# Itseez/opencv

Measured on AMD Instinct MI355X. Metric: Mpix/s per GPU (4K CV_8U Gaussian5x5) + achieved HBM GB/s vs roofline, 1/2/4/8 GPUs, higher is better.
Workload: dtype u8; 1 GPU; cv::GaussianBlur 5x5 sigma=0 BORDER_REFLECT_101 on 3840x2160 CV_8UC1, 9216 device-resident frames per GPU per step (152.9 GB of HBM: one pass = 18 launches of 512 frames); frames_per_gpu=9216, frames_per_launch=512, ranks=1, collective=none (1 GPU)

## Files before the change

opencv_amd/csrc/smooth.hip:

```cpp
#include "rt.h"
#include "gausskernel.h"
#include "seproll.h"
#include "seplong.h"
#include "sepmx.h"
#include <cstring>
#include <cstdlib>

using namespace mi355;

namespace {

struct FixedTaps { uint16_t kx[33]; uint16_t ky[33]; int nx, ny; };

__global__ __launch_bounds__(256) void k_sepfixed_generic(
    const uchar* __restrict__ src, size_t sstep, size_t sframe,
    uchar* __restrict__ dst, size_t dstep, size_t dframe,
    int W, int H, int cn, int mL, int mT, int mR, int mB, int border, FixedTaps t)
{
    const int b = blockIdx.x * 64 + (threadIdx.x & 63);
    const int y = blockIdx.y * 4 + (threadIdx.x >> 6);
    if (b >= W * cn || y >= H) return;
    src += (size_t)blockIdx.z * sframe;
    dst += (size_t)blockIdx.z * dframe;
    const int x = b / cn, c = b - x * cn;
// ... 119 lines not shown
                Hrow[k] = a + (b << 2) + (m << 1) + (m << 2); }
            {   uint32_t a = pairAt<1, -2 * CN, HD>(E, O, k) + pairAt<1, 2 * CN, HD>(E, O, k);
                uint32_t b = pairAt<1, -CN, HD>(E, O, k) + pairAt<1, CN, HD>(E, O, k);
                uint32_t m = pairAt<1, 0, HD>(E, O, k);
                Hrow[4 + k] = a + (b << 2) + (m << 1) + (m << 2); }
        } else {
            Hrow[k]     = pairAt<0, -CN, HD>(E, O, k) + pairAt<0, CN, HD>(E, O, k) + (pairAt<0, 0, HD>(E, O, k) << 1);
            Hrow[4 + k] = pairAt<1, -CN, HD>(E, O, k) + pairAt<1, CN, HD>(E, O, k) + (pairAt<1, 0, HD>(E, O, k) << 1);
        }
    }
}

template <int KS, int CN>
__global__ __launch_bounds__(256) void k_binomial_roll(
    const uchar* __restrict__ src, size_t sstep, size_t sframe,
    uchar* __restrict__ dst, size_t dstep, size_t dframe,
    int W, int H, int nchunks, int segRows, int border)
{
    constexpr int R = KS / 2, HD = RollCfg<KS, CN>::HD;
    const int lane = threadIdx.x & 63;
    const int c = (blockIdx.x * 4 + (threadIdx.x >> 6)) * 64 + lane;
    const int y0 = blockIdx.y * segRows;
    const int y1 = min(H, y0 + segRows);
    src += (size_t)blockIdx.z * sframe;
    dst += (size_t)blockIdx.z * dframe;
    const bool active = c < nchunks;

    uint32_t Hw[KS][8];
    {
        RawRow<HD> pre[KS - 1];
#pragma unroll
        for (int i = 0; i < KS - 1; i++) loadRow<KS, CN>(pre[i], src, sstep, y0 - R + i, W, H, c, nchunks, lane, border);
#pragma unroll
        for (int i = 0; i < KS - 1; i++) hfilter<KS, CN>(Hw[i], pre[i], c, nchunks, lane);
    }
    for (int y = y0; y < y1; y += KS) {
        RawRow<HD> raw[KS];
#pragma unroll
        for (int u = 0; u < KS; u++)
            if (y + u < y1) loadRow<KS, CN>(raw[u], src, sstep, y + u + R, W, H, c, nchunks, lane, border);
#pragma unroll
        for (int u = 0; u < KS; u++) {
            if (y + u < y1) {
                hfilter<KS, CN>(Hw[(KS - 1 + u) % KS], raw[u], c, nchunks, lane);
                uint32_t o[4];
                if constexpr (KS == 5) {
                    const uint32_t* h0 = Hw[(u + 0) % 5]; const uint32_t* h1 = Hw[(u + 1) % 5];
                    const uint32_t* h2 = Hw[(u + 2) % 5]; const uint32_t* h3 = Hw[(u + 3) % 5];
                    const uint32_t* h4 = Hw[(u + 4) % 5];
                    uint32_t v[8];
#pragma unroll
                    for (int i = 0; i < 8; i++) {
                        const uint32_t b4 = lshlAdd(h1[i] + h3[i] + h2[i], 2, 0x00800080u);
                        v[i] = h0[i] + h4[i] + lshlAdd(h2[i], 1, b4);
                    }
#pragma unroll
                    for (int k = 0; k < 4; k++) o[k] = __builtin_amdgcn_perm(v[4 + k], v[k], 0x07030501u);
                } else {
                    const uint32_t* h0 = Hw[(u + 0) % 3]; const uint32_t* h1 = Hw[(u + 1) % 3]; const uint32_t* h2 = Hw[(u + 2) % 3];
#pragma unroll
                    for (int k = 0; k < 4; k++) {
                        uint32_t ve = ((h0[k] + h2[k] + (h1[k] << 1) + 0x00080008u) >> 4) & 0x00FF00FFu;
                        uint32_t vo = ((h0[4 + k] + h2[4 + k] + (h1[4 + k] << 1) + 0x00080008u) >> 4) & 0x00FF00FFu;
                        o[k] = ve | (vo << 8);
                    }
                }
                if (active)
                    *reinterpret_cast<uint4*>(dst + (size_t)(y + u) * dstep + 16 * (size_t)c) = make_uint4(o[0], o[1], o[2], o[3]);
            }
        }
    }
}

template <int HD> struct RawRow2 {
    uint4 m;
    uint32_t side[HD];
};

template <int HD> struct EdgeSel {
    uint32_t la[HD], lb[HD], lc[HD];
    uint32_t ra[HD], rb[HD], rc[HD];
};

__device__ __forceinline__ void selSetByte(uint32_t& a, uint32_t& b, uint32_t& c, int j, int idx )
{
    const uint32_t sh = 8u * (uint32_t)j, clr = ~(0xffu << sh);
    uint32_t va = 0x0cu, vb = 0x0cu, vc = 0x0cu;
    if (idx >= 8)      { vb = (uint32_t)(idx - 8); vc = 4u + (uint32_t)j; }
    else if (idx >= 0) { va = (uint32_t)idx;       vc = (uint32_t)j; }
    a = (a & clr) | (va << sh); b = (b & clr) | (vb << sh); c = (c & clr) | (vc << sh);
}

__device__ __forceinline__ uint32_t gather16(const uint4& m, uint32_t a, uint32_t b, uint32_t c)
{
    const uint32_t t1 = __builtin_amdgcn_perm(m.y, m.x, a);
    const uint32_t t2 = __builtin_amdgcn_perm(m.w, m.z, b);
    return __builtin_amdgcn_perm(t2, t1, c);
}

template <int KS, int CN, bool NTL = false>
__device__ __forceinline__ void issueRow(RawRow2<RollCfg<KS, CN>::HD>& r, const uchar* __restrict__ row, int mainOff, int sideOff)
{
    constexpr int HD = RollCfg<KS, CN>::HD;
    if constexpr (NTL) {
        typedef uint32_t u32x4 __attribute__((ext_vector_type(4)));
        u32x4 v = __builtin_nontemporal_load(reinterpret_cast<const u32x4*>(row + mainOff));
        r.m = make_uint4(v.x, v.y, v.z, v.w);
    } else
    r.m = *reinterpret_cast<const uint4*>(row + mainOff);
#pragma unroll
    for (int d = 0; d < HD; d++) r.side[d] = *reinterpret_cast<const uint32_t*>(row + sideOff + 4 * d);
}

template <int KS, int CN, bool EB = true>
__device__ __forceinline__ void hfilter2(uint32_t (&Hrow)[8], const RawRow2<RollCfg<KS, CN>::HD>& r,
                                         bool hasFirst, bool hasLast, bool isLastChunk, const EdgeSel<RollCfg<KS, CN>::HD>& es)
{
    constexpr int HD = RollCfg<KS, CN>::HD;
    constexpr int NW = 4 + 2 * HD;
    uint32_t X[NW];
    const uint32_t mv[4] = {r.m.x, r.m.y, r.m.z, r.m.w};
    uint32_t hl[HD], hr[HD];
#pragma unroll
    for (int d = 0; d < HD; d++) { hl[d] = r.side[d]; hr[d] = r.side[d]; }
    if (hasFirst) {
#pragma unroll
        for (int d = 0; d < HD; d++) { hl[d] = gather16(r.m, es.la[d], es.lb[d], es.lc[d]); if constexpr (EB) asm volatile("" : "+v"(hl[d])); }
    }
    uint32_t hb[HD];
#pragma unroll
    for (int d = 0; d < HD; d++) hb[d] = 0;
    if (hasLast) {
#pragma unroll
        for (int d = 0; d < HD; d++) { hb[d] = gather16(r.m, es.ra[d], es.rb[d], es.rc[d]); if constexpr (EB) asm volatile("" : "+v"(hb[d])); }
    }
#pragma unroll
    for (int d = 0; d < HD; d++) {
        X[d] = __builtin_amdgcn_update_dpp(hl[d], mv[4 - HD + d], 0x138, 0xf, 0xf, false);
        uint32_t rr = __builtin_amdgcn_update_dpp(hr[d], mv[d], 0x130, 0xf, 0xf, false);
        if (hasLast) { rr = isLastChunk ? hb[d] : rr; if constexpr (EB) asm volatile("" : "+v"(rr)); }
        X[HD + 4 + d] = rr;
    }
#pragma unroll
    for (int d = 0; d < 4; d++) X[HD + d] = mv[d];
    uint32_t E[NW], O[NW];
#pragma unroll
    for (int d = 0; d < NW; d++) {
        E[d] = __builtin_amdgcn_perm(0u, X[d], 0x0c020c00u);
        O[d] = __builtin_amdgcn_perm(0u, X[d], 0x0c030c01u);
    }
#pragma unroll
    for (int k = 0; k < 4; k++) {
        if constexpr (KS == 5) {
            {   uint32_t a = pairAt<0, -2 * CN, HD>(E, O, k) + pairAt<0, 2 * CN, HD>(E, O, k);
                uint32_t b = pairAt<0, -CN, HD>(E, O, k) + pairAt<0, CN, HD>(E, O, k);
                uint32_t m = pairAt<0, 0, HD>(E, O, k);
                Hrow[k] = a + (b << 2) + (m << 1) + (m << 2); }
            {   uint32_t a = pairAt<1, -2 * CN, HD>(E, O, k) + pairAt<1, 2 * CN, HD>(E, O, k);
                uint32_t b = pairAt<1, -CN, HD>(E, O, k) + pairAt<1, CN, HD>(E, O, k);
                uint32_t m = pairAt<1, 0, HD>(E, O, k);
                Hrow[4 + k] = a + (b << 2) + (m << 1) + (m << 2); }
        } else {
            Hrow[k]     = pairAt<0, -CN, HD>(E, O, k) + pairAt<0, CN, HD>(E, O, k) + (pairAt<0, 0, HD>(E, O, k) << 1);
            Hrow[4 + k] = pairAt<1, -CN, HD>(E, O, k) + pairAt<1, CN, HD>(E, O, k) + (pairAt<1, 0, HD>(E, O, k) << 1);
        }
    }
}
// ... 105 lines not shown
            for (int k = 0; k < 4; k++) o[k] = __builtin_amdgcn_perm(v[4 + k], v[k], 0x07030501u);
        } else {
            const uint32_t* h0 = Hw[(u + 0) % 3]; const uint32_t* h1 = Hw[(u + 1) % 3]; const uint32_t* h2 = Hw[(u + 2) % 3];
#pragma unroll
            for (int k = 0; k < 4; k++) {
                uint32_t ve = ((h0[k] + h2[k] + (h1[k] << 1) + 0x00080008u) >> 4) & 0x00FF00FFu;
                uint32_t vo = ((h0[4 + k] + h2[4 + k] + (h1[4 + k] << 1) + 0x00080008u) >> 4) & 0x00FF00FFu;
                o[k] = ve | (vo << 8);
            }
        }
        if (active) {
            typedef uint32_t u32x4 __attribute__((ext_vector_type(4)));
            u32x4 ov = {o[0], o[1], o[2], o[3]};
            u32x4* dp = reinterpret_cast<u32x4*>(dst + (size_t)gy(j) * dstep + 16 * (size_t)c);
            if constexpr (NT) __builtin_nontemporal_store(ov, dp);
            else *dp = ov;
        }
    };
    if constexpr (RING) {
        RawRow2<HD> pre[KS - 1];
        int pvalid[KS - 1];
#pragma unroll
        for (int i = 0; i < KS - 1; i++) {
            const int ry = rowIdx(gy(min(i - R, nrows - 1 + R)));
            pvalid[i] = ry >= 0;
            issueRow<KS, CN>(pre[i], src + (size_t)max(ry, 0) * sstep, mainOff, sideOff);
            __builtin_amdgcn_sched_barrier(0);
        }
#pragma unroll
        for (int u = 0; u < KS; u++) {
            refill(u, u + R);
            __builtin_amdgcn_sched_barrier(0);
        }
#pragma unroll
        for (int i = 0; i < KS - 1; i++) {
            hfilter2<KS, CN, EB>(Hw[i], pre[i], hasFirst, hasLast, isLastChunk, es);
#pragma unroll
            for (int j = 0; j < 8; j++) Hw[i][j] = pvalid[i] ? Hw[i][j] : 0u;
        }
        int y = 0;
        for (; y + KS <= nrows; y += KS) {
#pragma unroll
            for (int u = 0; u < KS; u++) {
                consume(u);
                refill(u, y + u + KS + R);
                emit(u, y + u);
            }
        }
#pragma unroll
        for (int u = 0; u < KS - 1; u++) {
            if (y + u < nrows) {
                consume(u);
                emit(u, y + u);
            }
        }
    } else {
#pragma unroll
        for (int i = 0; i < KS - 1; i++) {
            const int ry = rowIdx(gy(min(i - R, nrows - 1 + R)));
            if (ry < 0) {
#pragma unroll
                for (int j = 0; j < 8; j++) Hw[i][j] = 0;
            } else {
                RawRow2<HD> pre;
                issueRow<KS, CN>(pre, src + (size_t)ry * sstep, mainOff, sideOff);
                hfilter2<KS, CN, EB>(Hw[i], pre, hasFirst, hasLast, isLastChunk, es);
            }
        }
#pragma unroll
        for (int u = 0; u < KS; u++) refill(u, u + R);
        for (int y = 0; y < nrows; y += KS) {
#pragma unroll
            for (int u = 0; u < KS; u++) {
                if (y + u < nrows) {
                    consume(u);
                    refill(u, y + u + KS + R);
                    emit(u, y + u);
                }
            }
        }
    }
}

template <bool NT>
__global__ __launch_bounds__(256) void k_copy16(const uint4* __restrict__ s, uint4* __restrict__ d, size_t n16, int perThread)
{
    typedef uint32_t u32x4 __attribute__((ext_vector_type(4)));
    size_t base = ((size_t)blockIdx.x * perThread) * 256 + threadIdx.x;
#pragma unroll 4
    for (int i = 0; i < perThread; i++) {
        size_t j = base + (size_t)i * 256;
        if (j < n16) {
            uint4 v = s[j];
            u32x4 ov = {v.x, v.y, v.z, v.w};
            if constexpr (NT) __builtin_nontemporal_store(ov, reinterpret_cast<u32x4*>(d + j));
            else d[j] = v;
        }
    }
}

template <int UNROLL>
__global__ __launch_bounds__(256) void k_copy_colwalk(const uchar* __restrict__ src, uchar* __restrict__ dst, size_t step, size_t frame,
                                                      int H, int nchunks, int nstrips, int segRows, int nseg, int nframes)
{
    const int lane = threadIdx.x & 63;
    const int wid = __builtin_amdgcn_readfirstlane((int)(blockIdx.x * 4 + (threadIdx.x >> 6)));
    const int strip = wid % nstrips, t0 = wid / nstrips, seg = t0 % nseg, fr = t0 / nseg;
    if (fr >= nframes) return;
    const int c = strip * 64 + lane;
    if (c >= nchunks) return;
    const int y0 = seg * segRows, y1 = min(H, y0 + segRows);
    const uchar* s = src + (size_t)fr * frame + 16 * (size_t)c;
    uchar* d = dst + (size_t)fr * frame + 16 * (size_t)c;
    for (int y = y0; y < y1; y += UNROLL) {
        uint4 v[UNROLL];
#pragma unroll
        for (int u = 0; u < UNROLL; u++) v[u] = *reinterpret_cast<const uint4*>(s + (size_t)min(y + u, y1 - 1) * step);
#pragma unroll
        for (int u = 0; u < UNROLL; u++) if (y + u < y1) *reinterpret_cast<uint4*>(d + (size_t)(y + u) * step) = v[u];
    }
}


bool aligned16(const void* p, size_t step) { return (((uintptr_t)p | step) & 15) == 0; }

int envInt(const char* n, int d) { const char* v = getenv(n); return v ? atoi(v) : d; }

int& tuneSeg() { static int v = envInt("MI355CV_GAUSS_SEG", 0); return v; }
constexpr int kGaussVariantDefault = 6;
int& tuneVariant() { static int v = envInt("MI355CV_GAUSS_VARIANT", kGaussVariantDefault); return v; }

int& tuneAlt() { static int v = envInt("MI355CV_GAUSS_ALT", 1); return v; }
int& tuneLaunchWaves() { static int v = envInt("MI355CV_GAUSS_LAUNCH_WAVES", 393216); return v; }

template <int KS, int CN>
void launchRoll2(const uchar* s, size_t ss, size_t sf, uchar* d, size_t ds, size_t df, int nframes, int W, int H, int border, hipStream_t st, int nt)
{
    const int nchunks = W * CN / 16;
    const int nstrips = divUp(nchunks, 64);
    int seg = tuneSeg();
    if (seg <= 0) {
        long long per = (long long)nstrips * nframes;
        long long wantSeg = (2048 + per - 1) / per;
        seg = (int)((H + wantSeg - 1) / wantSeg);
        const int best = (nt == 4 && CN == 1) ? 12 : 16;
        if (seg > best) seg = best;
        if (seg < KS) seg = KS;
    }
    if (seg > H) seg = H;
    const int nseg = divUp(H, seg);
    const long long perFrame = (long long)nstrips * nseg;
    long long chunk = tuneLaunchWaves() > 0 ? (tuneLaunchWaves() + perFrame - 1) / perFrame : nframes;
    if (chunk < 1) chunk = 1;
    if (chunk > nframes) chunk = nframes;
    const int nlaunch = (int)((nframes + chunk - 1) / chunk);
    noteKernel("k_binomial_roll2<%d,%d,%s,false,%d,%s%s> grid=%u x256 seg=%d rows alt=%d, %d launch(es) of <= %lld frames", KS, CN, nt >= 1 ? "true" : "false", nt == 3 ? 6 : 4,
               nt == 2 ? "false" : "true", nt == 4 ? ",true" : "", (unsigned)((perFrame * chunk + 3) / 4), seg, tuneAlt(), nlaunch, chunk);
    for (long long f0 = 0; f0 < nframes; f0 += chunk) {
        const int nf = (int)(nframes - f0 < chunk ? nframes - f0 : chunk);
        const uchar* sp = s + (size_t)f0 * sf;
        uchar* dp = d + (size_t)f0 * df;
        dim3 grid((unsigned)((perFrame * nf + 3) / 4));
        if (nt >= 4)      hipLaunchKernelGGL((k_binomial_roll2<KS, CN, true, false, 4, true, true>), grid, dim3(256), 0, st, sp, ss, sf, dp, ds, df, W, H, nchunks, nstrips, seg, nseg, nf, border, tuneAlt());
        else if (nt == 3) hipLaunchKernelGGL((k_binomial_roll2<KS, CN, true, false, 6>), grid, dim3(256), 0, st, sp, ss, sf, dp, ds, df, W, H, nchunks, nstrips, seg, nseg, nf, border, tuneAlt());
        else if (nt == 2) hipLaunchKernelGGL((k_binomial_roll2<KS, CN, true, false, 4, false>), grid, dim3(256), 0, st, sp, ss, sf, dp, ds, df, W, H, nchunks, nstrips, seg, nseg, nf, border, tuneAlt());
        else if (nt == 1) hipLaunchKernelGGL((k_binomial_roll2<KS, CN, true, false, 4>), grid, dim3(256), 0, st, sp, ss, sf, dp, ds, df, W, H, nchunks, nstrips, seg, nseg, nf, border, tuneAlt());
        else              hipLaunchKernelGGL((k_binomial_roll2<KS, CN, false, false, 4>), grid, dim3(256), 0, st, sp, ss, sf, dp, ds, df, W, H, nchunks, nstrips, seg, nseg, nf, border, tuneAlt());
    }
}

template <int KS, int CN>
void launchRoll(const uchar* s, size_t ss, size_t sf, uchar* d, size_t ds, size_t df, int nframes, int W, int H, int border, hipStream_t st)
{
    const int nchunks = W * CN / 16;
    const int gx = divUp(nchunks, 256);
    const int segEnv = tuneSeg();
    int seg;
    if (segEnv > 0) seg = segEnv;
    else {
        long long stripsWaves = (long long)divUp(nchunks, 64) * nframes;
        long long wantSeg = (16384 + stripsWaves - 1) / stripsWaves;
        if (wantSeg < 1) wantSeg = 1;
        seg = (int)((H + wantSeg - 1) / wantSeg);
        if (seg < 4 * KS) seg = 4 * KS;
    }
    seg = divUp(seg, KS) * KS;
    if (seg > H) seg = divUp(H, KS) * KS;
    for (int f0 = 0; f0 < nframes; f0 += MAX_GRID_FRAMES) {
        dim3 grid(gx, divUp(H, seg), std::min(MAX_GRID_FRAMES, nframes - f0));
        hipLaunchKernelGGL((k_binomial_roll<KS, CN>), grid, dim3(256), 0, st, s + (size_t)f0 * sf, ss, sf, d + (size_t)f0 * df, ds, df, W, H, nchunks, seg, border);
    }
    noteKernel("k_binomial_roll<%d,%d> grid=%dx%dx%d x256 seg=%d rows, %d launch(es)", KS, CN, gx, divUp(H, seg), std::min(MAX_GRID_FRAMES, nframes), seg, divUp(nframes, MAX_GRID_FRAMES));
}

bool rollEligible(const uchar* s, size_t ss, size_t sf, const uchar* d, size_t ds, size_t df, int W, int H, int cn, int ks)
{
    if (ks != 3 && ks != 5) return false;
    if (cn < 1 || cn > 4) return false;
    if (!aligned16(s, ss) || !aligned16(d, ds) || (sf & 15) || (df & 15)) return false;
    if ((W * cn) % 16 != 0) return false;
    if (H < 1) return false;
    return true;
}

static int sepmxMinTaps()
{
    static const int v = std::getenv("MI355CV_SEPMX_MIN_TAPS") ? atoi(std::getenv("MI355CV_SEPMX_MIN_TAPS")) : 7;
    return v;
}

int runSmooth(const char* entry, const uchar* src, size_t sstep, size_t sframe, uchar* dst, size_t dstep, size_t dframe,
              int nframes, int W, int H, int cn, int mL, int mT, int mR, int mB,
              const uint16_t* kx, int nx, const uint16_t* ky, int ny, int border, bool binomial)
{
    MI355_DECLINE_IF(disabled());
    MI355_DECLINE_IF(W <= 0 || H <= 0 || nframes <= 0 || cn < 1 || cn > 4);
    MI355_DECLINE_IF(nx < 1 || ny < 1 || nx > lim::GAUSS8U_MAX_KSIZE || ny > lim::GAUSS8U_MAX_KSIZE || !(nx & 1) || !(ny & 1));
    MI355_DECLINE_IF(border < 0 || border > B_REFLECT_101);
    Stager stg;
    MI355_DECLINE_IF(!ensureDevice());
    const bool hostSrc = !isDevicePtr(src);
    MI355_DECLINE_IF(hostSrc && (size_t)W * H < minPixels());
    MI355_DECLINE_IF(!hostSrc && src == dst);

    size_t dss = 0, dds = 0;
    const size_t rowB = (size_t)W * cn;
    const uchar* dsrc; uchar* ddst;
    if (nframes == 1) {
        const uchar* top = src - (ptrdiff_t)mT * (ptrdiff_t)sstep - (ptrdiff_t)mL * cn;
        const uchar* dtop = stg.in(top, sstep, (size_t)(mL + W + mR) * cn, mT + H + mB, &dss);
        MI355_DECLINE_IF(!dtop);
        dsrc = dtop + (size_t)mT * dss + (size_t)mL * cn;
        ddst = stg.out(dst, dstep, rowB, H, &dds);
        MI355_DECLINE_IF(!ddst);
    } else {
        if (hostSrc || !isDevicePtr(dst)) return setError(MI355CV_NOT_IMPLEMENTED, "%s: batch entry needs device-resident frames", entry);
        dsrc = src; ddst = dst; dss = sstep; dds = dstep;
    }
    hipStream_t st = stream();
    const bool noMargins = !(mL | mT | mR | mB);
    if (binomial && noMargins && rollEligible(dsrc, dss, sframe, ddst, dds, dframe, W, H, cn, nx) && nx == ny) {
#define ROLL(KS_, CN_) do { if (tuneVariant() <= 1 || border == B_WRAP || W <= KS_ / 2) launchRoll<KS_, CN_>(dsrc, dss, sframe, ddst, dds, dframe, nframes, W, H, border, st); \
                            else launchRoll2<KS_, CN_>(dsrc, dss, sframe, ddst, dds, dframe, nframes, W, H, border, st, tuneVariant() - 2); } while (0)
        if (nx == 5) { switch (cn) { case 1: ROLL(5, 1); break; case 2: ROLL(5, 2); break; case 3: ROLL(5, 3); break; default: ROLL(5, 4); } }
        else         { switch (cn) { case 1: ROLL(3, 1); break; case 2: ROLL(3, 2); break; case 3: ROLL(3, 3); break; default: ROLL(3, 4); } }
#undef ROLL
    } else if (std::getenv("MI355CV_SMOOTH_GENERIC") == nullptr && std::max(nx, ny) >= sepmxMinTaps() && !(std::getenv("MI355CV_SEPMX") && std::getenv("MI355CV_SEPMX")[0] == '0') &&
               sepmxRun(stg, dsrc, dss, sframe, ddst, dds, dframe, nframes, W, H, cn, mL + W + mR, mT + H + mB, mL, mT, border, kx, nx, nx / 2, ky, ny, ny / 2, st)) {
    } else if (noMargins && std::getenv("MI355CV_SMOOTH_GENERIC") == nullptr &&
               seprollFixedSmooth(dsrc, dss, sframe, ddst, dds, dframe, nframes, W, H, cn, kx, nx, ky, ny, border, st)) {
    } else if (!noMargins && nframes == 1 && std::getenv("MI355CV_SMOOTH_GENERIC") == nullptr && [&] {
                   const Roi roi = {mL + W + mR, mT + H + mB, mL, mT};
                   return seprollFixedSmooth(dsrc, dss, 0, ddst, dds, 0, 1, W, H, cn, kx, nx, ky, ny, border, st, &roi); }()) {
    } else if (std::getenv("MI355CV_SMOOTH_GENERIC") == nullptr && std::max(nx, ny) < sepmxMinTaps() && !(std::getenv("MI355CV_SEPMX") && std::getenv("MI355CV_SEPMX")[0] == '0') &&
               sepmxRun(stg, dsrc, dss, sframe, ddst, dds, dframe, nframes, W, H, cn, mL + W + mR, mT + H + mB, mL, mT, border, kx, nx, nx / 2, ky, ny, ny / 2, st)) {
    } else if (std::getenv("MI355CV_SMOOTH_GENERIC") == nullptr && [&] {
                   unsigned sx = 0, sy = 0;
                   for (int i = 0; i < nx; i++) sx += kx[i];
                   for (int i = 0; i < ny; i++) sy += ky[i];
                   if (sx > 256 || sy > 256) return false;
                   std::vector<int> ix(kx, kx + nx), iy(ky, ky + ny);
                   const SepLongTaps t = {nullptr, nullptr, ix.data(), iy.data(), nx, ny, nx / 2, ny / 2, 3, 0, 0.f, 0};
                   return seplongRun(stg, dsrc, dss, sframe, ddst, dds, dframe, nframes, W, H, cn, MI355CV_8U, MI355CV_8U, mL + W + mR, mT + H + mB, mL, mT, border, t, st); }()) {
    } else {
        MI355_DECLINE_IF((nx > 33 || ny > 33) && nframes > MAX_GRID_FRAMES);
        if (nx > 33 || ny > 33) return MI355_DECLINED("Q8.8 taps that sum beyond 256 with more than 33 of them");
        FixedTaps t;
        t.nx = nx; t.ny = ny;
        for (int i = 0; i < 33; i++) { t.kx[i] = i < nx ? kx[i] : 0; t.ky[i] = i < ny ? ky[i] : 0; }
        for (int f0 = 0; f0 < nframes; f0 += MAX_GRID_FRAMES) {
            dim3 grid(divUp(W * cn, 64), divUp(H, 4), std::min(MAX_GRID_FRAMES, nframes - f0));
            hipLaunchKernelGGL(k_sepfixed_generic, grid, dim3(256), 0, st, dsrc + (size_t)f0 * sframe, dss, sframe, ddst + (size_t)f0 * dframe, dds, dframe,
                               W, H, cn, mL, mT, mR, mB, border, t);
        }
        noteKernel("k_sepfixed_generic grid=%dx%dx%d x256, %d launch(es)", divUp(W * cn, 64), divUp(H, 4), std::min(MAX_GRID_FRAMES, nframes), divUp(nframes, MAX_GRID_FRAMES));
    }
    return stg.finish(entry);
}

template <int K>
__global__ __launch_bounds__(256) void k_binom16_direct(const uchar* __restrict__ parent, size_t sstep, uchar* __restrict__ dst, size_t dstep, int W, int H, int cn,
                                                        int mL, int mT, int fullW, int fullH, int border)
{
    constexpr int R = K / 2, SH = K == 3 ? 2 : K == 5 ? 4 : K == 7 ? 6 : 8;
    constexpr uint32_t TAP[9] = {K == 3 ? 1u : K == 5 ? 1u : K == 7 ? 2u : 4u, K == 3 ? 2u : K == 5 ? 4u : K == 7 ? 7u : 13u, K == 3 ? 1u : K == 5 ? 6u : K == 7 ? 14u : 30u,
                                 K == 5 ? 4u : K == 7 ? 18u : 51u, K == 5 ? 1u : K == 7 ? 14u : 60u, K == 7 ? 7u : 51u, K == 7 ? 2u : 30u, 13u, 4u};
    const int e = blockIdx.x * 64 + (threadIdx.x & 63), y = blockIdx.y * 4 + (threadIdx.x >> 6);
    if (e >= W * cn || y >= H) return;
    const int x = e / cn, c = e - x * cn;
    int xs[K];
#pragma unroll
    for (int i = 0; i < K; i++) { const int q = mi355_borderInterpolate(x + mL + i - R, fullW, border); xs[i] = q < 0 ? -1 : q * cn + c; }
    uint32_t acc = 0;
#pragma unroll
    for (int j = 0; j < K; j++) {
        const int q = mi355_borderInterpolate(y + mT + j - R, fullH, border);
        if (q < 0) continue;
        const unsigned short* row = reinterpret_cast<const unsigned short*>(parent + (size_t)q * sstep);
        uint32_t h = 0;
#pragma unroll
        for (int i = 0; i < K; i++) h += xs[i] < 0 ? 0u : TAP[i] * (uint32_t)row[xs[i]];
        acc += TAP[j] * h;
    }
    reinterpret_cast<unsigned short*>(dst + (size_t)y * dstep)[e] = (unsigned short)((acc + (1u << (2 * SH - 1))) >> (2 * SH));
}

int runBinom16(const char* entry, const uchar* src, size_t sstep, uchar* dst, size_t dstep, int W, int H, int cn, int mL, int mT, int mR, int mB, int ksize, int border)
{
    if (disabled() || W <= 0 || H <= 0 || cn < 1 || cn > 4 || (ksize != 3 && ksize != 5 && ksize != 7 && ksize != 9) || border < 0 || border > B_REFLECT_101 ||
        mL < 0 || mT < 0 || mR < 0 || mB < 0 || ((sstep | dstep | (uintptr_t)src | (uintptr_t)dst) & 1))
        return MI355_DECLINED("disabled() || W <= 0 || H <= 0 || cn < 1 || cn > 4 || ksize not in {3, 5, 7, 9} || border outside CONSTANT .. REFLECT_101 || negative margins || odd pointers / steps");
    Stager stg;
    MI355_DECLINE_IF(!ensureDevice());
    const bool hostSrc = !isDevicePtr(src);
    MI355_DECLINE_IF(hostSrc && (size_t)W * H < minPixels());
    MI355_DECLINE_IF(!hostSrc && src == dst);
    size_t dss = 0, dds = 0;
    const size_t esz = (size_t)cn * 2;
    const uchar* top = src - (ptrdiff_t)mT * (ptrdiff_t)sstep - (ptrdiff_t)mL * (ptrdiff_t)esz;
    const uchar* dtop = stg.in(top, sstep, (size_t)(mL + W + mR) * esz, mT + H + mB, &dss);
    MI355_DECLINE_IF(!dtop);
    const uchar* dsrc = dtop + (size_t)mT * dss + (size_t)mL * esz;
    uchar* ddst = stg.out(dst, dstep, (size_t)W * esz, H, &dds);
    MI355_DECLINE_IF(!ddst);
    const Roi roi = {mL + W + mR, mT + H + mB, mL, mT};
    if (cn == 1 && (ksize == 3 || ksize == 5) && border != B_WRAP &&
// ... 60 lines not shown
        return gaussBatchFromHost(src_data, src_step, src_frame_stride, dst_data, dst_step, dst_frame_stride, nframes, width, height, cn, k, (int)ksize,
                                  border_type & ~MI355CV_BORDER_ISOLATED);
    if (nframes == 1)
        return runSmooth("gaussianBlurBinomialBatch", src_data, src_step, 0, dst_data, dst_step, 0, 1, width, height, cn,
                         0, 0, 0, 0, k, (int)ksize, k, (int)ksize, border_type & ~MI355CV_BORDER_ISOLATED, true);
    return runSmooth("gaussianBlurBinomialBatch", src_data, src_step, src_frame_stride, dst_data, dst_step, dst_frame_stride,
                     nframes, width, height, cn, 0, 0, 0, 0, k, (int)ksize, k, (int)ksize,
                     border_type & ~MI355CV_BORDER_ISOLATED, true);
}

MI355CV_API int mi355cv_gaussianBlur(const uchar* src_data, size_t src_step, uchar* dst_data, size_t dst_step,
        int width, int height, int depth, int cn, size_t margin_left, size_t margin_top, size_t margin_right,
        size_t margin_bottom, size_t ksize_width, size_t ksize_height, double sigmaX, double sigmaY, int border_type)
{
    mi355::EntryGuard entry_(__func__);
    if (depth != MI355CV_8U) {
        if (depth != MI355CV_16U && depth != MI355CV_16S && depth != MI355CV_32F) return MI355_DECLINED("depth is none of 8U / 16U / 16S / 32F");
        const int n = (int)ksize_width, m = (int)ksize_height;
        if (n < 1 || m < 1 || n > lim::GAUSS_FLOAT_MAX_KSIZE || m > lim::GAUSS_FLOAT_MAX_KSIZE || !(n & 1) || !(m & 1)) return MI355_DECLINED("kernel size outside 1 .. lim::GAUSS_FLOAT_MAX_KSIZE or even");
        if (sigmaY <= 0) sigmaY = sigmaX;
        const double s1 = sigmaX > 0 ? sigmaX : 0, s2 = sigmaY > 0 ? sigmaY : 0;
        std::vector<double> dx, dy;
        MI355_DECLINE_IF(!gaussianKernelBitExact(n, s1, dx));
        if (m == n && std::fabs(s1 - s2) < 2.220446049250313e-16) dy = dx;
        else MI355_DECLINE_IF(!gaussianKernelBitExact(m, s2, dy));
        std::vector<float> fx(dx.begin(), dx.end()), fy(dy.begin(), dy.end());
        const int type = MI355CV_MAKETYPE(depth, cn);
        cvhalFilter2D* ctx = nullptr;
        int rc = mi355cv_sepFilterInit(&ctx, type, type, MI355CV_32F, reinterpret_cast<uchar*>(fx.data()), n, reinterpret_cast<uchar*>(fy.data()), m, -1, -1, 0.0, border_type);
        if (rc != MI355CV_OK) return rc;
        rc = mi355cv_sepFilter(ctx, const_cast<uchar*>(src_data), src_step, dst_data, dst_step, width, height, (int)(margin_left + (size_t)width + margin_right),
                               (int)(margin_top + (size_t)height + margin_bottom), (int)margin_left, (int)margin_top);
        (void)mi355cv_sepFilterFree(ctx);
        return rc;
    }
    if (margin_left | margin_top | margin_right | margin_bottom)
        return mi355::setError(MI355CV_NOT_IMPLEMENTED, "gaussianBlur: submatrix with real margins is the reference's sepFilter2D case");
    MI355_DECLINE_IF(ksize_width > (size_t)lim::GAUSS8U_MAX_KSIZE || ksize_height > (size_t)lim::GAUSS8U_MAX_KSIZE);
    if (sigmaY <= 0) sigmaY = sigmaX;
    std::vector<int64_t> qx, qy;
    MI355_DECLINE_IF(!gaussianKernelFixedQ((int)ksize_width, sigmaX > 0 ? sigmaX : 0, 8, qx));
    MI355_DECLINE_IF(!gaussianKernelFixedQ((int)ksize_height, sigmaY > 0 ? sigmaY : 0, 8, qy));
    uint16_t kx[lim::GAUSS8U_MAX_KSIZE], ky[lim::GAUSS8U_MAX_KSIZE];
    for (size_t i = 0; i < ksize_width; i++) { MI355_DECLINE_IF(qx[i] < 0 || qx[i] > 65535); kx[i] = (uint16_t)qx[i]; }
    for (size_t i = 0; i < ksize_height; i++) { MI355_DECLINE_IF(qy[i] < 0 || qy[i] > 65535); ky[i] = (uint16_t)qy[i]; }
    bool binom = ksize_width == ksize_height && (ksize_width == 3 || ksize_width == 5);
    if (binom) {
        const uint16_t* b = binomTaps(ksize_width);
        for (size_t i = 0; i < ksize_width; i++) if (kx[i] != b[i] || ky[i] != b[i]) binom = false;
    }
    return runSmooth("gaussianBlur", src_data, src_step, 0, dst_data, dst_step, 0, 1, width, height, cn,
                     (int)margin_left, (int)margin_top, (int)margin_right, (int)margin_bottom,
                     kx, (int)ksize_width, ky, (int)ksize_height, border_type & ~MI355CV_BORDER_ISOLATED, binom);
}

MI355CV_API int mi355cv_gaussianBlurBatch(const uchar* src_data, size_t src_step, size_t src_frame_stride, uchar* dst_data, size_t dst_step, size_t dst_frame_stride,
        int nframes, int width, int height, int depth, int cn, size_t ksize_width, size_t ksize_height, double sigmaX, double sigmaY, int border_type)
{
    mi355::EntryGuard entry_(__func__);
    MI355_DECLINE_IF(depth != MI355CV_8U);
    if (nframes < 1 || !(ksize_width & 1) || !(ksize_height & 1) || ksize_width > (size_t)lim::GAUSS8U_MAX_KSIZE || ksize_height > (size_t)lim::GAUSS8U_MAX_KSIZE)
        return MI355_DECLINED("nframes < 1 || even kernel size || ksize > lim::GAUSS8U_MAX_KSIZE");
    if (sigmaY <= 0) sigmaY = sigmaX;
    std::vector<int64_t> qx, qy;
    if (!gaussianKernelFixedQ((int)ksize_width, sigmaX > 0 ? sigmaX : 0, 8, qx) || !gaussianKernelFixedQ((int)ksize_height, sigmaY > 0 ? sigmaY : 0, 8, qy))
        return MI355_DECLINED("!gaussianKernelFixedQ");
    uint16_t kx[lim::GAUSS8U_MAX_KSIZE], ky[lim::GAUSS8U_MAX_KSIZE];
    for (size_t i = 0; i < ksize_width; i++) { MI355_DECLINE_IF(qx[i] < 0 || qx[i] > 65535); kx[i] = (uint16_t)qx[i]; }
    for (size_t i = 0; i < ksize_height; i++) { MI355_DECLINE_IF(qy[i] < 0 || qy[i] > 65535); ky[i] = (uint16_t)qy[i]; }
    bool binom = ksize_width == ksize_height && (ksize_width == 3 || ksize_width == 5);
    if (binom) {
        const uint16_t* b = binomTaps(ksize_width);
        for (size_t i = 0; i < ksize_width; i++) if (kx[i] != b[i] || ky[i] != b[i]) binom = false;
    }
    return runSmooth("gaussianBlurBatch", src_data, src_step, nframes > 1 ? src_frame_stride : 0, dst_data, dst_step, nframes > 1 ? dst_frame_stride : 0, nframes, width, height, cn,
                     0, 0, 0, 0, kx, (int)ksize_width, ky, (int)ksize_height, border_type & ~MI355CV_BORDER_ISOLATED, binom);
}

MI355CV_API int mi355cv_setParam(const char* key, int value)
{
    mi355::EntryGuard entry_(__func__);
    if (!key) return -1;
    if (!strcmp(key, "gauss_seg")) { tuneSeg() = value; return 0; }
    if (!strcmp(key, "gauss_variant")) { tuneVariant() = value > 0 ? value : kGaussVariantDefault; return 0; }
    if (!strcmp(key, "gauss_alt")) { tuneAlt() = value; return 0; }
    if (!strcmp(key, "gauss_launch_waves")) { tuneLaunchWaves() = value; return 0; }
    return -1;
}

MI355CV_API int mi355cv_copyProbe(const void* src, void* dst, size_t bytes, int perThread, int nt)
{
    mi355::EntryGuard entry_(__func__);
    MI355_DECLINE_IF(!ensureDevice() || (bytes & 15) || perThread < 1);
    size_t n16 = bytes / 16;
    size_t blocks = (n16 + (size_t)256 * perThread - 1) / ((size_t)256 * perThread);
    if (nt) hipLaunchKernelGGL((k_copy16<true>), dim3((unsigned)blocks), dim3(256), 0, stream(), (const uint4*)src, (uint4*)dst, n16, perThread);
    else    hipLaunchKernelGGL((k_copy16<false>), dim3((unsigned)blocks), dim3(256), 0, stream(), (const uint4*)src, (uint4*)dst, n16, perThread);
    if (hipGetLastError() != hipSuccess) return MI355CV_ERROR_UNKNOWN;
    if (!asyncMode()) (void)hipStreamSynchronize(stream());
    return MI355CV_OK;
}

MI355CV_API int mi355cv_copyProbeColwalk(const void* src, void* dst, int W, int H, int nframes, int segRows, int unroll)
{
    mi355::EntryGuard entry_(__func__);
    MI355_DECLINE_IF(!ensureDevice() || (W & 15));
    const int nchunks = W / 16, nstrips = divUp(nchunks, 64), nseg = divUp(H, segRows);
    const long long items = (long long)nstrips * nseg * nframes;
    dim3 grid((unsigned)((items + 3) / 4));
    const uchar* s = (const uchar*)src; uchar* d = (uchar*)dst;
    if (unroll == 1) hipLaunchKernelGGL((k_copy_colwalk<1>), grid, dim3(256), 0, stream(), s, d, (size_t)W, (size_t)W * H, H, nchunks, nstrips, segRows, nseg, nframes);
    else if (unroll == 2) hipLaunchKernelGGL((k_copy_colwalk<2>), grid, dim3(256), 0, stream(), s, d, (size_t)W, (size_t)W * H, H, nchunks, nstrips, segRows, nseg, nframes);
    else if (unroll == 5) hipLaunchKernelGGL((k_copy_colwalk<5>), grid, dim3(256), 0, stream(), s, d, (size_t)W, (size_t)W * H, H, nchunks, nstrips, segRows, nseg, nframes);
    else hipLaunchKernelGGL((k_copy_colwalk<10>), grid, dim3(256), 0, stream(), s, d, (size_t)W, (size_t)W * H, H, nchunks, nstrips, segRows, nseg, nframes);
    if (hipGetLastError() != hipSuccess) return MI355CV_ERROR_UNKNOWN;
    if (!asyncMode()) (void)hipStreamSynchronize(stream());
    return MI355CV_OK;
}

MI355CV_API int mi355cv_getGaussianKernelQ(int n, double sigma, int fractionBits, int64_t* taps)
{
    mi355::EntryGuard entry_(__func__);
    std::vector<int64_t> q;
    MI355_DECLINE_IF(!gaussianKernelFixedQ(n, sigma, fractionBits, q));
    for (int i = 0; i < n; i++) taps[i] = q[i];
    return MI355CV_OK;
}

MI355CV_API int mi355cv_getGaussianKernel(int n, double sigma, double* taps)
{
    mi355::EntryGuard entry_(__func__);
    std::vector<double> k;
    MI355_DECLINE_IF(!gaussianKernelBitExact(n, sigma, k));
    for (int i = 0; i < n; i++) taps[i] = k[i];
    return MI355CV_OK;
}

MI355CV_API int mi355cv_sepSmoothFixedU8(const uchar* src_data, size_t src_step, uchar* dst_data, size_t dst_step,
        int width, int height, int cn, size_t margin_left, size_t margin_top, size_t margin_right, size_t margin_bottom,
        const uint16_t* kx, int kxlen, const uint16_t* ky, int kylen, int border_type)
{
    mi355::EntryGuard entry_(__func__);
    MI355_DECLINE_IF(!kx || !ky);
    bool binom = kxlen == kylen && (kxlen == 3 || kxlen == 5);
    if (binom) {
        const uint16_t* b = binomTaps(kxlen);
        for (int i = 0; i < kxlen; i++) if (kx[i] != b[i] || ky[i] != b[i]) binom = false;
    }
    return runSmooth("sepSmoothFixedU8", src_data, src_step, 0, dst_data, dst_step, 0, 1, width, height, cn,
                     (int)margin_left, (int)margin_top, (int)margin_right, (int)margin_bottom,
                     kx, kxlen, ky, kylen, border_type & ~MI355CV_BORDER_ISOLATED, binom);
}

}
```

Measured before the change: 3.050 million Mpix/s.

## Add lean interior-segment roll kernel with precomputed plan and uniform addressing

Adds a new k_binomial_roll2 overload driven by a host-precomputed plan: edge selectors, magic-number division constants, segment alternation and border rows are all computed once on the host. Interior segments take a fast path with no per-row border remapping, SGPR-uniform global row pointers and a remainder count fixed at compile time. The default for wide 4K single-channel 5x5 now selects this lean variant with shorter segments. The cost is more template instantiations, a larger kernel-argument struct and a separate slower path kept for edge segments.

```diff
diff --git a/opencv_amd/csrc/smooth.hip b/opencv_amd/csrc/smooth.hip
--- a/opencv_amd/csrc/smooth.hip
+++ b/opencv_amd/csrc/smooth.hip
@@ -225,7 +225,7 @@
     uint32_t ra[HD], rb[HD], rc[HD];
 };
 
-__device__ __forceinline__ void selSetByte(uint32_t& a, uint32_t& b, uint32_t& c, int j, int idx )
+__host__ __device__ __forceinline__ void selSetByte(uint32_t& a, uint32_t& b, uint32_t& c, int j, int idx )
 {
     const uint32_t sh = 8u * (uint32_t)j, clr = ~(0xffu << sh);
     uint32_t va = 0x0cu, vb = 0x0cu, vc = 0x0cu;
@@ -497,6 +497,223 @@
     }
 }
 
+template <int HD> struct LeanPlanBase {
+    EdgeSel<HD> es;
+    int H, nchunks, nstrips, nseg, seg;
+    uint32_t mStrips, mSeg;
+    int lStrips, lSeg;
+    int altShift, altMask, altFull, pairFull, upMask;
+    int segLo, segHi;
+    int groups;
+    int rowAbove[2], rowBelow[2];
+};
+template <int HD, int REM> struct LeanPlan : LeanPlanBase<HD> { static constexpr int rem = REM; };
+
+template <int KS>
+__device__ __forceinline__ void vfilter2(uint32_t (&o)[4], const uint32_t (&Hw)[KS][8], int u)
+{
+    if constexpr (KS == 5) {
+        const uint32_t* h0 = Hw[(u + 0) % 5]; const uint32_t* h1 = Hw[(u + 1) % 5];
+        const uint32_t* h2 = Hw[(u + 2) % 5]; const uint32_t* h3 = Hw[(u + 3) % 5];
+        const uint32_t* h4 = Hw[(u + 4) % 5];
+        uint32_t v[8];
+#pragma unroll
+        for (int i = 0; i < 8; i++) {
+            const uint32_t b4 = lshlAdd(h1[i] + h3[i] + h2[i], 2, 0x00800080u);
+            v[i] = h0[i] + h4[i] + lshlAdd(h2[i], 1, b4);
+        }
+#pragma unroll
+        for (int k = 0; k < 4; k++) o[k] = __builtin_amdgcn_perm(v[4 + k], v[k], 0x07030501u);
+    } else {
+        const uint32_t* h0 = Hw[(u + 0) % 3]; const uint32_t* h1 = Hw[(u + 1) % 3]; const uint32_t* h2 = Hw[(u + 2) % 3];
+#pragma unroll
+        for (int k = 0; k < 4; k++) {
+            uint32_t ve = ((h0[k] + h2[k] + (h1[k] << 1) + 0x00080008u) >> 4) & 0x00FF00FFu;
+            uint32_t vo = ((h0[4 + k] + h2[4 + k] + (h1[4 + k] << 1) + 0x00080008u) >> 4) & 0x00FF00FFu;
+            o[k] = ve | (vo << 8);
+        }
+    }
+}
+
+#define MI355_GLOBAL_AS __attribute__((address_space(1)))
+template <class T>
+__device__ __forceinline__ MI355_GLOBAL_AS T* uniformGlobal(const void* p)
+{
+    const uint64_t v = (uint64_t)p;
+    const uint32_t lo = (uint32_t)__builtin_amdgcn_readfirstlane((int)(uint32_t)v), hi = (uint32_t)__builtin_amdgcn_readfirstlane((int)(uint32_t)(v >> 32));
+    return (MI355_GLOBAL_AS T*)(((uint64_t)hi << 32) | lo);
+}
+
+template <int KS, int CN>
+__device__ __forceinline__ void issueRowU(RawRow2<RollCfg<KS, CN>::HD>& r, const uchar* __restrict__ row, uint32_t mainOff, uint32_t sideOff)
+{
+    constexpr int HD = RollCfg<KS, CN>::HD;
+    typedef uint32_t u32x4 __attribute__((ext_vector_type(4)));
+    MI355_GLOBAL_AS const uchar* g = uniformGlobal<const uchar>(row);
+    const u32x4 v = *reinterpret_cast<MI355_GLOBAL_AS const u32x4*>(g + mainOff);
+    r.m = make_uint4(v.x, v.y, v.z, v.w);
+#pragma unroll
+    for (int d = 0; d < HD; d++) r.side[d] = *reinterpret_cast<MI355_GLOBAL_AS const uint32_t*>(g + sideOff + 4 * d);
+}
+
+template <int KS, int CN, class Plan>
+__global__ __launch_bounds__(256, 4) void k_binomial_roll2(
+    const uchar* __restrict__ src, size_t sstep, size_t sframe,
+    uchar* __restrict__ dst, size_t dstep, size_t dframe, int nitems, Plan p)
+{
+    constexpr int R = KS / 2, HD = RollCfg<KS, CN>::HD, REM = Plan::rem;
+    typedef uint32_t u32x4 __attribute__((ext_vector_type(4)));
+    const int lane = threadIdx.x & 63;
+    const uint32_t wid = (uint32_t)__builtin_amdgcn_readfirstlane((int)(blockIdx.x * 4 + (threadIdx.x >> 6)));
+    if (wid >= (uint32_t)nitems) return;
+    const uint32_t t0 = (__umulhi(wid, p.mStrips) + wid) >> p.lStrips;
+    const int strip = (int)(wid - t0 * (uint32_t)p.nstrips);
+    const uint32_t frame = (__umulhi(t0, p.mSeg) + t0) >> p.lSeg;
+    int seg = (int)(t0 - frame * (uint32_t)p.nseg);
+    if (seg < p.altFull) { const int j = seg & p.altMask; seg = seg - j + ((j & 7) << p.altShift) + (j >> 3); }
+    else if (seg < p.pairFull) { const int j = (seg - p.altFull) & 15; seg = seg - j + 2 * (j & 7) + (j >> 3); }
+    const int up = seg & p.upMask;
+    const int nchunks = p.nchunks;
+    const int c = strip * 64 + lane;
+    const int y0 = seg * p.seg;
+    src += (size_t)frame * sframe;
+    dst += (size_t)frame * dframe;
+    const bool active = c < nchunks;
+    const bool hasFirst = strip == 0, hasLast = strip == p.nstrips - 1;
+    const bool isLastChunk = c == nchunks - 1;
+    const int ce = active ? c : nchunks - 1;
+    const int mainOff = 16 * ce;
+    const int c0 = strip * 64;
+    const int leftOff = c0 > 0 ? 16 * c0 - 4 * HD : 0;
+    const int rightOff = c0 + 64 < nchunks ? 16 * (c0 + 64) : 16 * (nchunks - 1);
+    const int sideOff = lane < 32 ? leftOff : rightOff;
+    const uint32_t dstOff = 16u * (uint32_t)c;
+
+    uint32_t Hw[KS][8];
+    RawRow2<HD> raw[KS];
+    auto store = [&](uchar* drow, const uint32_t (&o)[4]) __attribute__((always_inline)) {
+        if (active) {
+            u32x4 ov = {o[0], o[1], o[2], o[3]};
+            __builtin_nontemporal_store(ov, reinterpret_cast<MI355_GLOBAL_AS u32x4*>(uniformGlobal<uchar>(drow) + dstOff));
+        }
+    };
+
+    if (seg >= p.segLo && seg < p.segHi) {
+        const ptrdiff_t sd = up ? -(ptrdiff_t)sstep : (ptrdiff_t)sstep, dd = up ? -(ptrdiff_t)dstep : (ptrdiff_t)dstep;
+        const uchar* sp = src + (size_t)(up ? y0 + p.seg - 1 + R : y0 - R) * sstep;
+        uchar* dp = dst + (size_t)(up ? y0 + p.seg - 1 : y0) * dstep;
+        RawRow2<HD> pre[KS - 1];
+#pragma unroll
+        for (int i = 0; i < KS - 1; i++) {
+            issueRowU<KS, CN>(pre[i], sp, (uint32_t)mainOff, (uint32_t)sideOff); sp += sd;
+            __builtin_amdgcn_sched_barrier(0);
+        }
+#pragma unroll
+        for (int u = 0; u < KS; u++) {
+            issueRowU<KS, CN>(raw[u], sp, (uint32_t)mainOff, (uint32_t)sideOff); sp += sd;
+            __builtin_amdgcn_sched_barrier(0);
+        }
+#pragma unroll
+        for (int i = 0; i < KS - 1; i++) hfilter2<KS, CN, true>(Hw[i], pre[i], hasFirst, hasLast, isLastChunk, p.es);
+        for (int g = 0; g < p.groups; g++) {
+#pragma unroll
+            for (int u = 0; u < KS; u++) {
+                hfilter2<KS, CN, true>(Hw[(KS - 1 + u) % KS], raw[u], hasFirst, hasLast, isLastChunk, p.es);
+                issueRowU<KS, CN>(raw[u], sp, (uint32_t)mainOff, (uint32_t)sideOff); sp += sd;
+                uint32_t o[4];
+                vfilter2<KS>(o, Hw, u);
+                store(dp, o); dp += dd;
+            }
+        }
+#pragma unroll
+        for (int u = 0; u < REM; u++) {
+            hfilter2<KS, CN, true>(Hw[(KS - 1 + u) % KS], raw[u], hasFirst, hasLast, isLastChunk, p.es);
+            issueRowU<KS, CN>(raw[u], sp, (uint32_t)mainOff, (uint32_t)sideOff); sp += sd;
+            uint32_t o[4];
+            vfilter2<KS>(o, Hw, u);
+            store(dp, o); dp += dd;
+        }
+#pragma unroll
+        for (int i = 0; i < KS; i++) {
+            const int u = (REM + i) % KS;
+            hfilter2<KS, CN, true>(Hw[(KS - 1 + u) % KS], raw[u], hasFirst, hasLast, isLastChunk, p.es);
+            uint32_t o[4];
+            vfilter2<KS>(o, Hw, u);
+            store(dp, o); dp += dd;
+        }
+        return;
+    }
+
+    const int H = p.H;
+    const int y1 = min(H, y0 + p.seg);
+    const int nrows = y1 - y0;
+    auto gy = [&](int j) -> int { return up ? y1 - 1 - j : y0 + j; };
+    auto rowIdx = [&](int g) -> int {
+        int ry = g;
+#pragma unroll
+        for (int i = 0; i < R; i++) { ry = (g == H + i) ? p.rowBelow[i] : ry; ry = (g == -1 - i) ? p.rowAbove[i] : ry; }
+        return ry;
+    };
+    int rvalid[KS];
+    auto consume = [&](int u) __attribute__((always_inline)) {
+        uint32_t (&Hn)[8] = Hw[(KS - 1 + u) % KS];
+        if (rvalid[u]) hfilter2<KS, CN, true>(Hn, raw[u], hasFirst, hasLast, isLastChunk, p.es);
+        else {
+#pragma unroll
+            for (int j = 0; j < 8; j++) Hn[j] = 0;
+        }
+    };
+    auto refill = [&](int u, int j) __attribute__((always_inline)) {
+        const int ry = rowIdx(gy(min(j, nrows - 1 + R)));
+        rvalid[u] = ry >= 0;
+        issueRow<KS, CN>(raw[u], src + (size_t)max(ry, 0) * sstep, mainOff, sideOff);
+    };
+    auto emit = [&](int u, int j) __attribute__((always_inline)) {
+        uint32_t o[4];
+        vfilter2<KS>(o, Hw, u);
+        if (active) {
+            u32x4 ov = {o[0], o[1], o[2], o[3]};
+            __builtin_nontemporal_store(ov, reinterpret_cast<u32x4*>(dst + (size_t)gy(j) * dstep + 16 * (size_t)c));
+        }
+    };
+    RawRow2<HD> pre[KS - 1];
+    int pvalid[KS - 1];
+#pragma unroll
+    for (int i = 0; i < KS - 1; i++) {
+        const int ry = rowIdx(gy(min(i - R, nrows - 1 + R)));
+        pvalid[i] = ry >= 0;
+        issueRow<KS, CN>(pre[i], src + (size_t)max(ry, 0) * sstep, mainOff, sideOff);
+        __builtin_amdgcn_sched_barrier(0);
+    }
+#pragma unroll
+    for (int u = 0; u < KS; u++) {
+        refill(u, u + R);
+        __builtin_amdgcn_sched_barrier(0);
+    }
+#pragma unroll
+    for (int i = 0; i < KS - 1; i++) {
+        hfilter2<KS, CN, true>(Hw[i], pre[i], hasFirst, hasLast, isLastChunk, p.es);
+#pragma unroll
+        for (int j = 0; j < 8; j++) Hw[i][j] = pvalid[i] ? Hw[i][j] : 0u;
+    }
+    int y = 0;
+    for (; y + KS <= nrows; y += KS) {
+#pragma unroll
+        for (int u = 0; u < KS; u++) {
+            consume(u);
+            refill(u, y + u + KS + R);
+            emit(u, y + u);
+        }
+    }
+#pragma unroll
+    for (int u = 0; u < KS - 1; u++) {
+        if (y + u < nrows) {
+            consume(u);
+            emit(u, y + u);
+        }
+    }
+}
+
 template <bool NT>
 __global__ __launch_bounds__(256) void k_copy16(const uint4* __restrict__ s, uint4* __restrict__ d, size_t n16, int perThread)
 {
@@ -542,33 +759,110 @@
 int envInt(const char* n, int d) { const char* v = getenv(n); return v ? atoi(v) : d; }
 
 int& tuneSeg() { static int v = envInt("MI355CV_GAUSS_SEG", 0); return v; }
-constexpr int kGaussVariantDefault = 6;
-int& tuneVariant() { static int v = envInt("MI355CV_GAUSS_VARIANT", kGaussVariantDefault); return v; }
+constexpr int kGaussVariantDefault = 7;
+int& tuneVariant() { static int v = envInt("MI355CV_GAUSS_VARIANT", 0); return v; }
 
 int& tuneAlt() { static int v = envInt("MI355CV_GAUSS_ALT", 1); return v; }
 int& tuneLaunchWaves() { static int v = envInt("MI355CV_GAUSS_LAUNCH_WAVES", 393216); return v; }
 
+void exactDiv(uint32_t d, uint32_t& m, int& l)
+{
+    l = 0;
+    while ((1ull << l) < d) l++;
+    m = (uint32_t)(((1ull << 32) * ((1ull << l) - d)) / d + 1);
+}
+
 template <int KS, int CN>
-void launchRoll2(const uchar* s, size_t ss, size_t sf, uchar* d, size_t ds, size_t df, int nframes, int W, int H, int border, hipStream_t st, int nt)
+LeanPlanBase<RollCfg<KS, CN>::HD> makeLeanPlan(int W, int H, int nchunks, int nstrips, int seg, int nseg, int border, int alt)
+{
+    constexpr int R = KS / 2, HD = RollCfg<KS, CN>::HD, HB = RollCfg<KS, CN>::HB;
+    LeanPlanBase<HD> p = {};
+    EdgeSel<HD>& es = p.es;
+    for (int d = 0; d < HD; d++) { es.la[d] = es.lb[d] = es.lc[d] = es.ra[d] = es.rb[d] = es.rc[d] = 0x0c0c0c0cu; }
+    for (int t = 0; t < HB; t++) {
+        const int bt = t - HB;
+        const int px = (bt - (CN - 1)) / CN;
+        const int sp = mi355_borderInterpolate(px, W, border);
+        const int pos = 4 * HD - HB + t;
+        selSetByte(es.la[pos >> 2], es.lb[pos >> 2], es.lc[pos >> 2], pos & 3, sp < 0 ? -1 : sp * CN + (bt - px * CN));
+    }
+    for (int t = 0; t < HB; t++) {
+        const int sp = mi355_borderInterpolate(W + t / CN, W, border);
+        selSetByte(es.ra[t >> 2], es.rb[t >> 2], es.rc[t >> 2], t & 3, sp < 0 ? -1 : sp * CN + (t % CN) - 16 * (nchunks - 1));
+    }
+    p.H = H; p.nchunks = nchunks; p.nstrips = nstrips; p.nseg = nseg; p.seg = seg;
+    exactDiv((uint32_t)nstrips, p.mStrips, p.lStrips);
+    exactDiv((uint32_t)nseg, p.mSeg, p.lSeg);
+    if (alt > 0) {
+        const int a = std::min(alt, 20), span = 8 << a;
+        p.altShift = a; p.altMask = span - 1; p.upMask = 1;
+        p.altFull = nseg / span * span;
+        p.pairFull = a > 1 ? p.altFull + (nseg - p.altFull) / 16 * 16 : p.altFull;
+    }
+    if (seg >= KS && H >= R) { p.segLo = (R + seg - 1) / seg; p.segHi = (H - R) / seg; }
+    p.groups = seg / KS - 1;
+    for (int i = 0; i < R; i++) { p.rowBelow[i] = mi355_borderInterpolate(H + i, H, border); p.rowAbove[i] = mi355_borderInterpolate(-1 - i, H, border); }
+    return p;
+}
+
+template <int KS, int CN, int REM>
+void launchLean(const LeanPlanBase<RollCfg<KS, CN>::HD>& base, dim3 grid, hipStream_t st, const uchar* s, size_t ss, size_t sf, uchar* d, size_t ds, size_t df, int nitems)
+{
+    LeanPlan<RollCfg<KS, CN>::HD, REM> p;
+    static_cast<LeanPlanBase<RollCfg<KS, CN>::HD>&>(p) = base;
+    hipLaunchKernelGGL((k_binomial_roll2<KS, CN, LeanPlan<RollCfg<KS, CN>::HD, REM>>), grid, dim3(256), 0, st, s, ss, sf, d, ds, df, nitems, p);
+}
+
+template <int KS, int CN>
+void launchRoll2(const uchar* s, size_t ss, size_t sf, uchar* d, size_t ds, size_t df, int nframes, int W, int H, int border, hipStream_t st, int variant)
 {
     const int nchunks = W * CN / 16;
     const int nstrips = divUp(nchunks, 64);
+    const bool wide = nstrips >= 4;
+    const bool byDefault = variant <= 0;
+    int nt = (byDefault ? ((KS == 5 && CN == 1 && !wide) ? 6 : kGaussVariantDefault) : variant) - 2;
     int seg = tuneSeg();
     if (seg <= 0) {
         long long per = (long long)nstrips * nframes;
         long long wantSeg = (2048 + per - 1) / per;
         seg = (int)((H + wantSeg - 1) / wantSeg);
-        const int best = (nt == 4 && CN == 1) ? 12 : 16;
+        const int lean = CN == 1 ? (KS == 3 ? (wide ? 4 : 6) : (wide ? 7 : 10)) : (KS == 3 ? 7 : 12);
+        const int best = nt >= 5 ? lean : (nt == 4 && CN == 1) ? 12 : 16;
         if (seg > best) seg = best;
         if (seg < KS) seg = KS;
     }
     if (seg > H) seg = H;
     const int nseg = divUp(H, seg);
+    if (byDefault && nt >= 5 && !(seg >= KS && (H - KS / 2) / seg > (KS / 2 + seg - 1) / seg)) nt = 4;
     const long long perFrame = (long long)nstrips * nseg;
     long long chunk = tuneLaunchWaves() > 0 ? (tuneLaunchWaves() + perFrame - 1) / perFrame : nframes;
     if (chunk < 1) chunk = 1;
     if (chunk > nframes) chunk = nframes;
+    if (nt >= 5 && perFrame * chunk > 0x7fffffffLL) chunk = std::max(1LL, 0x7fffffffLL / perFrame);
     const int nlaunch = (int)((nframes + chunk - 1) / chunk);
+    if (nt >= 5) {
+        const auto plan = makeLeanPlan<KS, CN>(W, H, nchunks, nstrips, seg, nseg, border, tuneAlt());
+        noteKernel("k_binomial_roll2<%d,%d,lean%d> grid=%u x256 seg=%d rows alt=%d, %d launch(es) of <= %lld frames", KS, CN, seg % KS,
+                   (unsigned)((perFrame * chunk + 3) / 4), seg, tuneAlt(), nlaunch, chunk);
+        for (long long f0 = 0; f0 < nframes; f0 += chunk) {
+            const int nf = (int)(nframes - f0 < chunk ? nframes - f0 : chunk);
+            const uchar* sp = s + (size_t)f0 * sf;
+            uchar* dp = d + (size_t)f0 * df;
+            const int nitems = (int)(perFrame * nf);
+            dim3 grid((unsigned)((perFrame * nf + 3) / 4));
+            switch (seg % KS) {
+            case 0: launchLean<KS, CN, 0>(plan, grid, st, sp, ss, sf, dp, ds, df, nitems); break;
+            case 1: launchLean<KS, CN, 1>(plan, grid, st, sp, ss, sf, dp, ds, df, nitems); break;
+            case 2: launchLean<KS, CN, 2>(plan, grid, st, sp, ss, sf, dp, ds, df, nitems); break;
+            default:
+                if constexpr (KS == 5) {
+                    if (seg % KS == 3) launchLean<KS, CN, 3>(plan, grid, st, sp, ss, sf, dp, ds, df, nitems);
+                    else               launchLean<KS, CN, 4>(plan, grid, st, sp, ss, sf, dp, ds, df, nitems);
+                }
+            }
+        }
+        return;
+    }
     noteKernel("k_binomial_roll2<%d,%d,%s,false,%d,%s%s> grid=%u x256 seg=%d rows alt=%d, %d launch(es) of <= %lld frames", KS, CN, nt >= 1 ? "true" : "false", nt == 3 ? 6 : 4,
                nt == 2 ? "false" : "true", nt == 4 ? ",true" : "", (unsigned)((perFrame * chunk + 3) / 4), seg, tuneAlt(), nlaunch, chunk);
     for (long long f0 = 0; f0 < nframes; f0 += chunk) {
@@ -655,8 +949,8 @@
     hipStream_t st = stream();
     const bool noMargins = !(mL | mT | mR | mB);
     if (binomial && noMargins && rollEligible(dsrc, dss, sframe, ddst, dds, dframe, W, H, cn, nx) && nx == ny) {
-#define ROLL(KS_, CN_) do { if (tuneVariant() <= 1 || border == B_WRAP || W <= KS_ / 2) launchRoll<KS_, CN_>(dsrc, dss, sframe, ddst, dds, dframe, nframes, W, H, border, st); \
-                            else launchRoll2<KS_, CN_>(dsrc, dss, sframe, ddst, dds, dframe, nframes, W, H, border, st, tuneVariant() - 2); } while (0)
+#define ROLL(KS_, CN_) do { if (tuneVariant() == 1 || border == B_WRAP || W <= KS_ / 2) launchRoll<KS_, CN_>(dsrc, dss, sframe, ddst, dds, dframe, nframes, W, H, border, st); \
+                            else launchRoll2<KS_, CN_>(dsrc, dss, sframe, ddst, dds, dframe, nframes, W, H, border, st, tuneVariant()); } while (0)
         if (nx == 5) { switch (cn) { case 1: ROLL(5, 1); break; case 2: ROLL(5, 2); break; case 3: ROLL(5, 3); break; default: ROLL(5, 4); } }
         else         { switch (cn) { case 1: ROLL(3, 1); break; case 2: ROLL(3, 2); break; case 3: ROLL(3, 3); break; default: ROLL(3, 4); } }
 #undef ROLL
@@ -883,7 +1177,7 @@
     mi355::EntryGuard entry_(__func__);
     if (!key) return -1;
     if (!strcmp(key, "gauss_seg")) { tuneSeg() = value; return 0; }
-    if (!strcmp(key, "gauss_variant")) { tuneVariant() = value > 0 ? value : kGaussVariantDefault; return 0; }
+    if (!strcmp(key, "gauss_variant")) { tuneVariant() = value > 0 ? value : 0; return 0; }
     if (!strcmp(key, "gauss_alt")) { tuneAlt() = value; return 0; }
     if (!strcmp(key, "gauss_launch_waves")) { tuneLaunchWaves() = value; return 0; }
     return -1;
```

New measurement: 3.075 million Mpix/s (median of 6 runs). Within noise of the previous version (+0.8%).
